# endernewton/tf-faster-rcnn

Hardware: NVIDIA H100
Metric: images/sec (higher is better)
Workload: dtype f16x3 (fp32-grade: fp16 hi/lo split of both operands, 3 wgmma f16 MMAs per product, fp32 accumulate)

## Files before the change

### include/frcnn_b200.h

```cpp
#ifndef FRCNN_B200_H_
#define FRCNN_B200_H_

#include <stddef.h>
#include <stdint.h>

#ifdef __cplusplus
extern "C" {
#endif

typedef enum {
  FRCNN_OK = 0,
  FRCNN_ERR_CUDA = -1,
  FRCNN_ERR_ARG = -2,
  FRCNN_ERR_NO_DEVICE = -3,
  FRCNN_ERR_DRIVER_ENTRY = -4,
  FRCNN_ERR_CAPACITY = -5
} frcnn_status;

#define FRCNN_NMS_PLUS_ONE 1u
#define FRCNN_NMS_INCLUSIVE 2u
#define FRCNN_NMS_SKIP_DEGENERATE 4u
#define FRCNN_NMS_MODE_CPU_NMS (FRCNN_NMS_PLUS_ONE | FRCNN_NMS_INCLUSIVE)
#define FRCNN_NMS_MODE_GPU_NMS (FRCNN_NMS_PLUS_ONE)
#define FRCNN_NMS_MODE_TF (FRCNN_NMS_SKIP_DEGENERATE)
// ... 1 lines not shown
#define FRCNN_ACT_NONE 0
#define FRCNN_ACT_RELU 1
#define FRCNN_ACT_RELU6 2

int frcnn_version(void);
int frcnn_last_error(char* buf, size_t buflen);
int frcnn_check_device(int device_id);
int frcnn_zero_async(void* dev_ptr, size_t bytes, void* stream);

typedef struct frcnn_graph frcnn_graph;
int frcnn_graph_begin(void* stream);
int frcnn_graph_end(void* stream, frcnn_graph** out);
int frcnn_graph_launch(const frcnn_graph* g, void* stream);
void frcnn_graph_destroy(frcnn_graph* g);

int frcnn_nms_host(int* keep_out, int* num_out, const float* boxes_host, int boxes_num, int boxes_dim,
                   float nms_overlap_thresh, int device_id, unsigned flags);

int frcnn_nms_sorted_dev(const float* boxes_dev, int n, float thresh, unsigned flags, int max_out,
                         int* keep_dev, int* num_dev, void* stream);

typedef struct frcnn_conv_plan frcnn_conv_plan;
#define FRCNN_CONV_F16X3 0
#define FRCNN_CONV_TF32X3 1
#define FRCNN_CONV_F16X1 2

typedef struct {
  const float* in_dev;
  const void* w_hi_dev;
  const void* w_lo_dev;
  const float* scale_dev;
  const float* shift_dev;
  const float* residual_dev;
  float* out_dev;
  int n, h, w, cin;
  int cout, kh, kw, stride;
  int pad_t, pad_l;
  int ho, wo;
  int act;
  int block_n;
  int kb_per_chunk;
  int split_k;
  int impl;
  float out_mult;
  const float* in2_dev;
  int cin2;
  float* mean_dev;
  int mean_hw;
} frcnn_conv_desc;

int frcnn_conv_plan_create(frcnn_conv_plan** out, const frcnn_conv_desc* d);
int frcnn_conv_plan_run(const frcnn_conv_plan* p, void* stream);
int frcnn_conv_plan_geometry(const frcnn_conv_desc* d, int sm_count, int* out16);
int frcnn_conv_plan_info(const frcnn_conv_plan* p, int* block_n, int* tile_n, int* tile_h, int* tile_w,
                         int* grid_m, int* grid_n, int* splits, int* smem_bytes);
int frcnn_conv_plan_set_trace(frcnn_conv_plan* p, long long* trace_dev);
void frcnn_conv_plan_destroy(frcnn_conv_plan* p);
int frcnn_debug_watchdog(unsigned int* out16, int reset);

int frcnn_pack_conv_weights(const float* w_hwio_dev, void* w_hi_dev, void* w_lo_dev, int kh, int kw,
                            int cin, int cout, int wexp, void* stream);
int frcnn_pack_conv_weights_tf32(const float* w_hwio_dev, float* w_hi_dev, float* w_lo_dev, int kh, int kw,
                                 int cin, int cout, void* stream);

int frcnn_conv_first(const float* in_dev, const float* w_hwio_dev, const float* scale_dev,
                     const float* shift_dev, float* out_dev, int n, int h, int w, int cout, int k,
                     int stride, int pad_t, int pad_l, int ho, int wo, int act, void* stream);
int frcnn_depthwise3x3(const float* in_dev, const float* w_dev, const float* scale_dev,
                       const float* shift_dev, float* out_dev, int n, int h, int w, int c, int stride,
                       int pad_t, int pad_l, int ho, int wo, int act, void* stream);
int frcnn_max_pool(const float* in_dev, float* out_dev, int n, int h, int w, int c, int k, int stride,
                   int pad_t, int pad_l, int ho, int wo, int pad_is_neg_inf, void* stream);
int frcnn_spatial_mean(const float* in_dev, float* out_dev, int r, int hw, int c, void* stream);

int frcnn_preprocess(const unsigned char* img_dev, int h0, int w0, const double* means3, double fx, double fy,
                     float* blob_dev, int H, int W, void* stream);
int frcnn_preprocess_hflip(const unsigned char* img_dev, int h0, int w0, const double* means3, double fx, double fy,
                           float* blob_dev, int H, int W, void* stream);


int frcnn_rpn_decode(const float* rpn_out_dev, int ld, int delta_col, const float* base_anchors_dev, int num_anchors,
                     int batch, int fh, int fw, int feat_stride, float im_h, float im_w, float* scores_dev,
                     float* props_dev, void* stream);
size_t frcnn_sort_workspace_bytes(int n);
int frcnn_sort_desc(const float* keys_dev, int n, int batch, int* order_dev, float* sorted_keys_dev, void* workspace_dev,
                    size_t workspace_bytes, void* stream);
int frcnn_proposals(const float* props_dev, const float* scores_dev, const int* order_dev, int n, int batch,
                    int pre_nms_top_n, int post_nms_top_n, float thresh, unsigned flags, float* rois_dev,
                    float* roi_scores_dev, int* keep_dev, int* num_dev, void* stream);
int frcnn_crop_pool(const float* feat_dev, int batch, int fh, int fw, int c, const float* rois_dev, int r, int pooled,
                    int pre_pool, float* out_dev, void* stream);
#define FRCNN_ROI_ALIGN_MAX_SAMPLING 16
int frcnn_roi_align(const float* feat_dev, int batch, int fh, int fw, int c, const float* rois_dev, int r, int pooled,
                    float spatial_scale, int sampling_ratio, int aligned, float* out_dev, void* stream);
int frcnn_roi_pool(const float* feat_dev, int batch, int fh, int fw, int c, const float* rois_dev, int r, int pooled,
                   float spatial_scale, float* out_dev, void* stream);
int frcnn_cls_finish(const float* head_out_dev, int ld, int r, int num_classes, const float* stds4,
                     const float* means4, float* cls_score_dev, float* cls_prob_dev, float* bbox_pred_dev,
                     void* stream);
int frcnn_bbox_decode(const float* rois_dev, const float* bbox_pred_dev, int r, int num_classes, int batch,
                      const float* im_meta_dev, float* pred_boxes_dev, void* stream);
size_t frcnn_detect_post_workspace_bytes(int r, int num_classes, int batch);
int frcnn_detect_post(const float* cls_prob_dev, const float* pred_boxes_dev, const int* num_rois_dev, int r, int batch,
                      int num_classes, float score_thresh, float nms_thresh, unsigned flags,
                      int max_per_image, int max_det, float* det_dev, int* ndet_dev, int record_stride, int* keep_dev,
                      int* keep_cnt_dev, float* keep_score_dev, void* workspace_dev, size_t workspace_bytes, void* stream);
// ... 53 lines not shown
```

### tf_faster_rcnn_b200/_native.py

```python
import ctypes as C
import os

_HERE = os.path.dirname(os.path.abspath(__file__))
LIB_PATH = os.path.join(_HERE, "libfrcnn_b200_wd.so" if os.environ.get("FRCNN_LIB_VARIANT") == "wd" else "libfrcnn_b200.so")

NMS_PLUS_ONE, NMS_INCLUSIVE, NMS_SKIP_DEGENERATE = 1, 2, 4
NMS_MODE_CPU_NMS = NMS_PLUS_ONE | NMS_INCLUSIVE
NMS_MODE_GPU_NMS = NMS_PLUS_ONE
NMS_MODE_TF = NMS_SKIP_DEGENERATE
ACT_NONE, ACT_RELU, ACT_RELU6 = 0, 1, 2
CONV_F16X3, CONV_TF32X3, CONV_F16X1 = 0, 1, 2
SOFT_NMS_METHODS = {"linear": 0, "gaussian": 1, "hard": 2}
AUG_MAX_VIEWS = 16
BOX_VOTE_METHODS = {"ID": 0, "AVG": 1, "IOU_AVG": 2, "GENERALIZED_AVG": 3, "QUASI_SUM": 4, "TEMP_AVG": 5}
ROI_ALIGN_MAX_SAMPLING = 16
ROI_MAX_POOLED = 16

vp, ci, cf, cu, sz = C.c_void_p, C.c_int, C.c_float, C.c_uint, C.c_size_t
ip, fp = C.POINTER(C.c_int), C.POINTER(C.c_float)


class ConvDesc(C.Structure):
    _fields_ = [("in_dev", vp), ("w_hi_dev", vp), ("w_lo_dev", vp), ("scale_dev", vp), ("shift_dev", vp),
                ("residual_dev", vp), ("out_dev", vp),
                ("n", ci), ("h", ci), ("w", ci), ("cin", ci), ("cout", ci), ("kh", ci), ("kw", ci), ("stride", ci),
                ("pad_t", ci), ("pad_l", ci), ("ho", ci), ("wo", ci), ("act", ci), ("block_n", ci), ("kb_per_chunk", ci), ("split_k", ci),
                ("impl", ci), ("out_mult", cf), ("in2_dev", vp), ("cin2", ci), ("mean_dev", vp), ("mean_hw", ci)]


SIGNATURES = {
    "frcnn_version": (ci, []),
    "frcnn_last_error": (ci, [C.c_char_p, sz]),
    "frcnn_check_device": (ci, [ci]),
    "frcnn_zero_async": (ci, [vp, sz, vp]),
    "frcnn_graph_begin": (ci, [vp]),
    "frcnn_graph_end": (ci, [vp, C.POINTER(vp)]),
    "frcnn_graph_launch": (ci, [vp, vp]),
    "frcnn_graph_destroy": (None, [vp]),
    "frcnn_nms_host": (ci, [ip, ip, fp, ci, ci, cf, ci, cu]),
    "frcnn_nms_sorted_dev": (ci, [vp, ci, cf, cu, ci, vp, vp, vp]),
    "frcnn_conv_plan_create": (ci, [C.POINTER(vp), C.POINTER(ConvDesc)]),
    "frcnn_conv_plan_run": (ci, [vp, vp]),
    "frcnn_conv_plan_geometry": (ci, [C.POINTER(ConvDesc), ci, ip]),
    "frcnn_conv_plan_info": (ci, [vp, ip, ip, ip, ip, ip, ip, ip, ip]),
    "frcnn_conv_plan_set_trace": (ci, [vp, vp]),
    "frcnn_conv_plan_destroy": (None, [vp]),
    "frcnn_debug_watchdog": (ci, [C.POINTER(C.c_uint), ci]),
    "frcnn_pack_conv_weights": (ci, [vp, vp, vp, ci, ci, ci, ci, ci, vp]),
    "frcnn_pack_conv_weights_tf32": (ci, [vp, vp, vp, ci, ci, ci, ci, vp]),
    "frcnn_conv_first": (ci, [vp, vp, vp, vp, vp, ci, ci, ci, ci, ci, ci, ci, ci, ci, ci, ci, vp]),
    "frcnn_depthwise3x3": (ci, [vp, vp, vp, vp, vp, ci, ci, ci, ci, ci, ci, ci, ci, ci, ci, vp]),
    "frcnn_max_pool": (ci, [vp, vp, ci, ci, ci, ci, ci, ci, ci, ci, ci, ci, ci, vp]),
    "frcnn_spatial_mean": (ci, [vp, vp, ci, ci, ci, vp]),
    "frcnn_preprocess": (ci, [vp, ci, ci, C.POINTER(C.c_double), C.c_double, C.c_double, vp, ci, ci, vp]),
    "frcnn_rpn_decode": (ci, [vp, ci, ci, vp, ci, ci, ci, ci, ci, cf, cf, vp, vp, vp]),
    "frcnn_sort_workspace_bytes": (sz, [ci]),
    "frcnn_sort_desc": (ci, [vp, ci, ci, vp, vp, vp, sz, vp]),
    "frcnn_proposals": (ci, [vp, vp, vp, ci, ci, ci, ci, cf, cu, vp, vp, vp, vp, vp]),
    "frcnn_crop_pool": (ci, [vp, ci, ci, ci, ci, vp, ci, ci, ci, vp, vp]),
    "frcnn_roi_align": (ci, [vp, ci, ci, ci, ci, vp, ci, ci, cf, ci, ci, vp, vp]),
    "frcnn_roi_pool": (ci, [vp, ci, ci, ci, ci, vp, ci, ci, cf, vp, vp]),
    "frcnn_cls_finish": (ci, [vp, ci, ci, ci, fp, fp, vp, vp, vp, vp]),
    "frcnn_bbox_decode": (ci, [vp, vp, ci, ci, ci, vp, vp, vp]),
    "frcnn_detect_post_workspace_bytes": (sz, [ci, ci, ci]),
    "frcnn_detect_regions_workspace_bytes": (ci, [ci, ci, ci, C.POINTER(sz)]),
    "frcnn_detect_post": (ci, [vp, vp, vp, ci, ci, ci, cf, cf, cu, ci, ci, vp, vp, ci, vp, vp, vp, vp, sz, vp]),
    "frcnn_soft_nms_host": (ci, [fp, ip, ip, fp, ci, ci, ci, cf, cf, cf, ci]),
    "frcnn_detect_post_soft": (ci, [vp, vp, vp, ci, ci, ci, cf, ci, cf, cf, cf, ci, ci, vp, vp, ci, vp, vp, vp, vp, sz, vp]),
    "frcnn_detect_features": (ci, [vp, vp, vp, ci, ci, ci, ci, ci, vp, vp, vp]),
    "frcnn_detect_regions": (ci, [vp, vp, vp, vp, vp, ci, ci, ci, ci, cf, cu, cf, ci, ci, vp, vp, vp, vp, sz, vp, vp, vp, vp, vp, vp, vp,
                                  vp, vp]),
    "frcnn_regions_attr_embed": (ci, [vp, ci, ci, ci, vp, vp, ci, vp, ci, vp, vp]),
    "frcnn_attr_finish": (ci, [vp, ci, ci, ci, ci, vp, vp, vp, vp, vp]),
    "frcnn_boxes_to_rois": (ci, [vp, vp, vp, ci, ci, vp, vp, vp]),
    "frcnn_preprocess_hflip": (ci, [vp, ci, ci, C.POINTER(C.c_double), C.c_double, C.c_double, vp, ci, ci, vp]),
    "frcnn_aug_union": (ci, [C.POINTER(vp), C.POINTER(vp), C.POINTER(vp), ip, ip, ci, ci, ci, vp, vp, vp, vp, vp]),
    "frcnn_box_vote_host": (ci, [fp, fp, ci, ci, fp, ci, ci, cf, ci, cf, ci]),
    "frcnn_detect_post_vote": (ci, [vp, vp, vp, ci, ci, ci, cf, cf, cu, ci, ci, vp, vp, ci, vp, vp, vp, vp, sz, cf, ci, cf, vp, vp]),
    "frcnn_detect_post_soft_vote": (ci, [vp, vp, vp, ci, ci, ci, cf, ci, cf, cf, cf, ci, ci, vp, vp, ci, vp, vp, vp, vp, sz, cf, ci, cf, vp,
                                         vp]),
}

_lib = None


def lib():
    global _lib
    if _lib is None:
        if not os.path.exists(LIB_PATH):
            raise RuntimeError("libfrcnn_b200.so not built (%s): the CUDA extension is mandatory, "
                               "there is no CPU fallback" % LIB_PATH)
        L = C.CDLL(LIB_PATH)
        for name, (res, args) in SIGNATURES.items():
            fn = getattr(L, name)
            fn.restype = res
            fn.argtypes = args
# ... 14 lines not shown
```

### tf_faster_rcnn_b200/csrc/conv_gemm.cu

```cuda
#include <cuda_fp16.h>
#include "common.cuh"
#include "../../include/frcnn_b200.h"
#include <stdlib.h>
#include <string.h>

namespace frcnn {

constexpr int BLOCK_M = 128;
constexpr int BLOCK_K = 32;
constexpr int A_TILE_BYTES = BLOCK_M * BLOCK_K * 4;
constexpr int NUM_CONSUMERS = 256;
constexpr int NUM_THREADS = NUM_CONSUMERS + 128;
constexpr int REGS_PRODUCER = 40, REGS_CONSUMER = 232;
constexpr int STAGES = 3;

struct ConvKernelParams {
  float* out;
  const float* residual;
  const float* scale;
  const float* shift;
  int cout, ho, wo, nimg;
  int tn, th, tw;
  int tiles_h, tiles_w;
  int kh, kw, cin, stride, pad_t, pad_l;
  int act;
  int a_box_bytes;
  int kb_per_split;
  int m_tiles, n_tiles, total_units, n_full, splits;
  int raster_n;
  float* ws;
  long long* trace;
  int num_kb_total;
  int cin2;
  float* mean_out;
  float* mean_ws;
  int mean_hw, mean_segs, mean_ld;
};

#ifdef FRCNN_WATCHDOG
#define FRCNN_TRACE(slot, kbv)                                                              \
  do {                                                                                      \
    if (p.trace && blockIdx.x == 0 && (kbv) < 64) p.trace[(kbv) * 8 + (slot)] = clock64(); \
  } while (0)
#else
#define FRCNN_TRACE(slot, kbv) do { } while (0)
#endif

template <int MODE> struct KTraits {
  static constexpr bool TF32 = MODE == FRCNN_CONV_TF32X3;
  static constexpr bool X1 = MODE == FRCNN_CONV_F16X1;
  static constexpr int BOXES = TF32 ? 1 : 2;
  static constexpr int A_BYTES = BOXES * A_TILE_BYTES;
  static constexpr float LO_SCALE = TF32 ? 1.f : 0.00048828125f;
};
template <int BN> constexpr int b_plane_bytes() { return BN * 128; }
template <int BN, int MODE> constexpr int stage_bytes() { return KTraits<MODE>::A_BYTES + 2 * b_plane_bytes<BN>(); }
template <int BN, int MODE> constexpr int smem_bytes() {
  return STAGES * stage_bytes<BN, MODE>() + 1024  + 64 ;
}
constexpr int MEAN_COLS = 64, MEAN_LD = MEAN_COLS + 2;
constexpr int MEAN_SMEM = BLOCK_M * MEAN_LD * 4;
static_assert(smem_bytes<128, FRCNN_CONV_F16X3>() + MEAN_SMEM <= 227 * 1024, "ring exceeds the sm_90 shared-memory limit per block");

struct Unit {
  int w0, h0, n0, nblk, z, kb0, num_kb, slot;
};
__device__ __forceinline__ Unit decode_unit(const ConvKernelParams& p, int u, int num_kb_total) {
  Unit t;
  int tile;
  if (u < p.n_full) { tile = u; t.z = 0; t.slot = -1; }
  else { const int v = u - p.n_full; t.slot = v / p.splits; t.z = v - t.slot * p.splits; tile = p.n_full + t.slot; }
  int mt;
  if (p.raster_n) { t.nblk = tile % p.n_tiles; mt = tile / p.n_tiles; }
  else { mt = tile % p.m_tiles; t.nblk = tile / p.m_tiles; }
  const int tile_w = mt % p.tiles_w;
  const int tile_h = (mt / p.tiles_w) % p.tiles_h;
  const int tile_n = mt / (p.tiles_w * p.tiles_h);
  t.w0 = tile_w * p.tw; t.h0 = tile_h * p.th; t.n0 = tile_n * p.tn;
  if (t.slot < 0) { t.kb0 = 0; t.num_kb = num_kb_total; }
  else { t.kb0 = t.z * p.kb_per_split; t.num_kb = min(p.kb_per_split, num_kb_total - t.kb0); }
  return t;
}

template <int ACT>
__device__ __forceinline__ float apply_act(float a) {
  if (ACT == FRCNN_ACT_RELU) return fmaxf(a, 0.f);
  if (ACT == FRCNN_ACT_RELU6) return fminf(fmaxf(a, 0.f), 6.f);
  return a;
}

template <bool RES, int ACT>
__device__ __forceinline__ float2 finish2(const float2 v, const float2 sc, const float2 sh, const float2 r) {
  float2 y;
  y.x = __fadd_rn(__fmul_rn(v.x, sc.x), sh.x); y.y = __fadd_rn(__fmul_rn(v.y, sc.y), sh.y);
  if (RES) { y.x = __fadd_rn(y.x, r.x); y.y = __fadd_rn(y.y, r.y); }
  y.x = apply_act<ACT>(y.x); y.y = apply_act<ACT>(y.y);
  return y;
}

constexpr int EPI_CHUNK = 8;
template <int BN, bool RES, int ACT>
__device__ __forceinline__ void epilogue_vec(const ConvKernelParams& p, const float (&acc)[BN / 2], const int cbase,
                                             const int pix0, const int pix1) {
  const int cout = p.cout;
  constexpr int NJ = BN / 8;
  constexpr int CH = NJ < EPI_CHUNK ? NJ : EPI_CHUNK;
  static_assert(NJ % CH == 0, "chunking");
  const float* const res0 = RES ? p.residual + (size_t)(pix0 >= 0 ? pix0 : 0) * cout : nullptr;
  const float* const res1 = RES ? p.residual + (size_t)(pix1 >= 0 ? pix1 : 0) * cout : nullptr;
#pragma unroll
  for (int j0 = 0; j0 < NJ; j0 += CH) {
    if (cbase + 8 * j0 >= cout) break;
    float2 sc[CH], sh[CH], r0[CH], r1[CH];
#pragma unroll
    for (int jj = 0; jj < CH; ++jj) {
      const int c = cbase + 8 * (j0 + jj);
      sc[jj] = ld_nc_f2_pinned(p.scale + c);
      sh[jj] = ld_nc_f2_pinned(p.shift + c);
      if (RES) {
        r0[jj] = ld_nc_f2_pinned_if(res0 + c, pix0 >= 0 && c < cout);
        r1[jj] = ld_nc_f2_pinned_if(res1 + c, pix1 >= 0 && c < cout);
      } else {
        r0[jj] = r1[jj] = sc[jj];
      }
    }
#pragma unroll
    for (int jj = 0; jj < CH; ++jj) {
      const int j = j0 + jj;
      const int c = cbase + 8 * j;
      if (c >= cout) break;
      if (pix0 >= 0)
        *reinterpret_cast<float2*>(p.out + (size_t)pix0 * cout + c) =
            finish2<RES, ACT>(make_float2(acc[4 * j], acc[4 * j + 1]), sc[jj], sh[jj], r0[jj]);
      if (pix1 >= 0)
// ... 80 lines not shown
      }
      *reinterpret_cast<float2*>(buf + r0 * MEAN_LD + 8 * jj + 2 * q4) = y0;
      *reinterpret_cast<float2*>(buf + (r0 + 8) * MEAN_LD + 8 * jj + 2 * q4) = y1;
    }
    consumer_bar();
    for (int s = tid / MEAN_COLS; s < nseg; s += NUM_CONSUMERS / MEAN_COLS) {
      const int g = g0 + s;
      const int rs = max(g * hw - t.w0, 0), re = min((g + 1) * hw - t.w0, nrows);
      const float* b = buf + col;
      float a0 = b[rs * MEAN_LD], a1 = 0.f, a2 = 0.f, a3 = 0.f;
      int r = rs + 1;
      for (; r + 3 < re; r += 4) {
        a1 = __fadd_rn(a1, b[r * MEAN_LD]); a2 = __fadd_rn(a2, b[(r + 1) * MEAN_LD]);
        a3 = __fadd_rn(a3, b[(r + 2) * MEAN_LD]); a0 = __fadd_rn(a0, b[(r + 3) * MEAN_LD]);
      }
      for (; r < re; ++r) a1 = __fadd_rn(a1, b[r * MEAN_LD]);
      p.mean_ws[((size_t)mt * p.mean_segs + s) * ld + (size_t)t.nblk * BN + cc + col] = __fadd_rn(__fadd_rn(a0, a1), __fadd_rn(a2, a3));
    }
  }
}

template <int BN>
__device__ __forceinline__ void epilogue_tile(const ConvKernelParams& p, const Unit& t, const float (&acc)[BN / 2], int r0, int q4,
                                              float* mean_buf) {
  if (p.mean_out) {
    epilogue_mean<BN>(p, t, acc, r0, q4, mean_buf);
    return;
  }
  if (t.slot >= 0) {
    float* const w = p.ws + ((size_t)t.slot * p.splits + t.z) * (size_t)(BLOCK_M * BN) + 2 * q4;
#pragma unroll
    for (int j = 0; j < BN / 8; ++j) {
      __stcg(reinterpret_cast<float2*>(w + (size_t)r0 * BN + 8 * j), make_float2(acc[4 * j], acc[4 * j + 1]));
      __stcg(reinterpret_cast<float2*>(w + (size_t)(r0 + 8) * BN + 8 * j), make_float2(acc[4 * j + 2], acc[4 * j + 3]));
    }
    return;
  }
  const int pix0 = tile_pixel(p, t, r0), pix1 = tile_pixel(p, t, r0 + 8);
  const int cbase = t.nblk * BN + 2 * q4;
  if ((p.cout & 3) != 0) {
    epilogue_generic<BN>(p, acc, cbase, pix0, pix1);
    return;
  }
  if (p.residual) epilogue_dispatch<BN, true>(p, acc, cbase, pix0, pix1);
  else epilogue_dispatch<BN, false>(p, acc, cbase, pix0, pix1);
}

template <int BN, int MODE>
__device__ __forceinline__ void wgmma_rs(float (&d)[BN / 2], const uint32_t (&a)[4], uint64_t b_desc, uint32_t scale_d) {
  if (KTraits<MODE>::TF32) wgmma_tf32_rs<BN>(d, a, b_desc, scale_d);
  else wgmma_f16_rs<BN>(d, a, b_desc, scale_d);
}

template <int BN, int MODE>
__global__ void __launch_bounds__(NUM_THREADS, 1)
conv_gemm_kernel(const __grid_constant__ CUtensorMap tmA, const __grid_constant__ CUtensorMap tmA2,
                 const __grid_constant__ CUtensorMap tmBhi, const __grid_constant__ CUtensorMap tmBlo, const ConvKernelParams p) {
  using T = KTraits<MODE>;
  constexpr int kStage = stage_bytes<BN, MODE>();
  constexpr int kPlane = b_plane_bytes<BN>();
  constexpr int NACC = BN / 2;
  static_assert(BN == 64 || BN == 128, "block_n");

  extern __shared__ uint8_t smem_raw[];
  uint8_t* smem = reinterpret_cast<uint8_t*>((reinterpret_cast<uintptr_t>(smem_raw) + 1023) & ~uintptr_t(1023));
  uint64_t* full = reinterpret_cast<uint64_t*>(smem + STAGES * kStage);
  uint64_t* empty = full + STAGES;

  const int warp = threadIdx.x >> 5;
  const int lane = threadIdx.x & 31;
  const int num_kb_total = p.num_kb_total;

  if (threadIdx.x == NUM_CONSUMERS) {
    tma_prefetch_desc(&tmA); tma_prefetch_desc(&tmBhi); tma_prefetch_desc(&tmBlo);
    if (p.cin2) tma_prefetch_desc(&tmA2);
    for (int s = 0; s < STAGES; ++s) { mbar_init(&full[s], 1); mbar_init(&empty[s], NUM_CONSUMERS); }
    mbar_fence_init();
  }
  __syncthreads();
  pdl_launch_dependents();
  pdl_wait();

  if (warp >= NUM_CONSUMERS / 32) {
    reg_dec<REGS_PRODUCER>();
    if (warp == NUM_CONSUMERS / 32 && lane == 0) {
      const int cchunks = p.cin / BLOCK_K;
      const int total1 = p.kh * p.kw * cchunks;
      const int cchunks2 = p.cin2 / BLOCK_K;
      const uint32_t tx = (uint32_t)(T::BOXES * p.a_box_bytes + (T::X1 ? 1 : 2) * kPlane);
      int s = 0; uint32_t ph = 0, kbt = 0;
      for (int u = blockIdx.x; u < p.total_units; u += gridDim.x) {
        const Unit t = decode_unit(p, u, num_kb_total);
#pragma unroll 1
        for (int kb = 0; kb < t.num_kb; ++kb, ++kbt) {
          MBAR_WAIT(&empty[s], ph ^ 1u, 4, kbt);
          uint8_t* st = smem + s * kStage;
          mbar_expect_tx(&full[s], tx);
#pragma unroll
          for (int i = 0; i < T::BOXES; ++i) {
            const int g32 = (t.kb0 + kb) * T::BOXES + i;
            int tap = g32 / cchunks, kc = g32 - tap * cchunks;
            const CUtensorMap* ma = &tmA;
            if (g32 >= total1) {
              tap = 0;
              if (cchunks2) { ma = &tmA2; kc = min(g32 - total1, cchunks2); }
              else kc = cchunks;
            }
            const int r = tap / p.kw, sx = tap - r * p.kw;
            tma_load_4d(st + i * A_TILE_BYTES, ma, &full[s], kc * BLOCK_K, t.w0 * p.stride + sx - p.pad_l,
                        t.h0 * p.stride + r - p.pad_t, t.n0);
          }
          const int kcoord = (t.kb0 + kb) * T::BOXES * BLOCK_K;
          tma_load_2d(st + T::A_BYTES, &tmBhi, &full[s], kcoord, t.nblk * BN);
          if (!T::X1) tma_load_2d(st + T::A_BYTES + kPlane, &tmBlo, &full[s], kcoord, t.nblk * BN);
          FRCNN_TRACE(0, kbt);
          if (++s == STAGES) { s = 0; ph ^= 1u; }
        }
      }
    }
    return;
  }

  reg_inc<REGS_CONSUMER>();
  const int wg = warp >> 2;
  const int q4 = lane & 3;
  const int r0 = wg * 64 + (warp & 3) * 16 + (lane >> 2);
  const uint32_t swz = (uint32_t)(lane >> 2);
  uint32_t aoff[4][2];
#pragma unroll
  for (int j = 0; j < 4; ++j)
#pragma unroll
    for (int h = 0; h < 2; ++h) {
      const int ch = T::TF32 ? j * 8 + h * 4 + q4 : (j & 1) * 16 + h * 8 + 2 * q4;
      const int box = T::TF32 ? 0 : j >> 1;
      aoff[j][h] = (uint32_t)(box * A_TILE_BYTES + r0 * 128) + ((((uint32_t)ch >> 2) ^ swz) << 4) + (((uint32_t)ch & 3u) << 2);
    }
  const uint32_t smem0 = smem_u32(smem);
  int s = 0; uint32_t ph = 0, kbt = 0;
  for (int u = blockIdx.x; u < p.total_units; u += gridDim.x) {
    const Unit t = decode_unit(p, u, num_kb_total);
    float acc[NACC], part[NACC];
#pragma unroll
    for (int i = 0; i < NACC; ++i) { acc[i] = 0.f; part[i] = 0.f; }
#pragma unroll 1
    for (int kb = 0; kb < t.num_kb; ++kb, ++kbt) {
      MBAR_WAIT(&full[s], ph, 1, kbt);
      if (threadIdx.x == 0) FRCNN_TRACE(1, kbt);
      const uint32_t sa = smem0 + (uint32_t)(s * kStage);
      uint32_t ahi[4][4], alo[4][4];
#pragma unroll
      for (int j = 0; j < 4; ++j) {
#pragma unroll
        for (int f = 0; f < 4; ++f) {
          const uint32_t addr = sa + aoff[j][f >> 1] + ((f & 1) ? 1024u : 0u);
          if (T::TF32) {
            float x;
            asm volatile("ld.shared.f32 %0, [%1];" : "=f"(x) : "r"(addr));
            const float hi = to_tf32(x);
            ahi[j][f] = __float_as_uint(hi);
            alo[j][f] = __float_as_uint(to_tf32_fast(__fsub_rn(x, hi)));
          } else {
            float2 x;
            asm volatile("ld.shared.v2.f32 {%0, %1}, [%2];" : "=f"(x.x), "=f"(x.y) : "r"(addr));
            const uint32_t h = pack_f16x2_rn(x.x, x.y);
            const float2 fh = __half22float2(*reinterpret_cast<const __half2*>(&h));
            ahi[j][f] = h;
            alo[j][f] = T::X1 ? 0u : pack_f16x2_rn(__fmul_rn(__fsub_rn(x.x, fh.x), 2048.f), __fmul_rn(__fsub_rn(x.y, fh.y), 2048.f));
          }
        }
      }
      const uint64_t bhi = wgmma_sw128_desc(sa + (uint32_t)T::A_BYTES);
      const uint64_t blo = wgmma_sw128_desc(sa + (uint32_t)(T::A_BYTES + kPlane));
#pragma unroll
      for (int i = 0; i < NACC; ++i) reg_fence(part[i]);
      wgmma_fence();
#pragma unroll
      for (int j = 0; j < 4; ++j) wgmma_rs<BN, MODE>(part, ahi[j], bhi + 2u * j, j > 0 ? 1u : 0u);
      wgmma_commit();
      wgmma_wait_all();
#pragma unroll
      for (int i = 0; i < NACC; ++i) { reg_fence(part[i]); acc[i] = __fadd_rn(acc[i], part[i]); }
      if (!T::X1) {
        wgmma_fence();
#pragma unroll
        for (int j = 0; j < 4; ++j) {
          wgmma_rs<BN, MODE>(part, alo[j], bhi + 2u * j, j > 0 ? 1u : 0u);
          wgmma_rs<BN, MODE>(part, ahi[j], blo + 2u * j, 1u);
        }
        wgmma_commit();
        wgmma_wait_all();
#pragma unroll
        for (int i = 0; i < NACC; ++i) { reg_fence(part[i]); acc[i] = __fmaf_rn(part[i], T::LO_SCALE, acc[i]); }
      }
      mbar_arrive(&empty[s]);
      if (threadIdx.x == 0) FRCNN_TRACE(2, kbt);
      if (++s == STAGES) { s = 0; ph ^= 1u; }
    }
    epilogue_tile<BN>(p, t, acc, r0, q4, reinterpret_cast<float*>(full + 8));
  }
}

template <int BN>
__global__ void __launch_bounds__(256)
tail_reduce_kernel(const ConvKernelParams p) {
  pdl_launch_dependents();
  pdl_wait();
  constexpr int RPB = 256 / (BN / 4);
  constexpr int GROUPS = BLOCK_M / RPB;
  const int slot = blockIdx.x / GROUPS, rgroup = blockIdx.x % GROUPS;
  const int tile = p.n_full + slot;
  const int mt = p.raster_n ? tile / p.n_tiles : tile % p.m_tiles, nblk = p.raster_n ? tile % p.n_tiles : tile / p.m_tiles;
  const int tile_w = mt % p.tiles_w, tile_h = (mt / p.tiles_w) % p.tiles_h, tile_n = mt / (p.tiles_w * p.tiles_h);
  const int rows_img = p.th * p.tw;
  constexpr int C4 = BN / 4;
  static_assert(256 % C4 == 0, "each thread keeps one fixed channel group");
  const float* base = p.ws + (size_t)slot * p.splits * (size_t)(BLOCK_M * BN);
  const bool vec_ok = (p.cout & 3) == 0;
  const int cg = threadIdx.x % C4;
  const int c = nblk * BN + cg * 4;
  if (c >= p.cout) return;
  const float4 sc4 = __ldg(reinterpret_cast<const float4*>(p.scale + c)), sh4 = __ldg(reinterpret_cast<const float4*>(p.shift + c));
  const float sc[4] = {sc4.x, sc4.y, sc4.z, sc4.w}, sh[4] = {sh4.x, sh4.y, sh4.z, sh4.w};
  {
    const int row = rgroup * RPB + threadIdx.x / C4;
    const int dn = row / rows_img, rem = row % rows_img;
    const int n = tile_n * p.tn + dn, h = tile_h * p.th + rem / p.tw, w = tile_w * p.tw + rem % p.tw;
    if (row >= p.tn * rows_img || n >= p.nimg || h >= p.ho || w >= p.wo) return;
    const size_t o = ((((size_t)n * p.ho + h) * p.wo + w)) * p.cout + c;
    float4 rv = make_float4(0.f, 0.f, 0.f, 0.f);
    if (p.residual) {
      if (vec_ok) rv = __ldg(reinterpret_cast<const float4*>(p.residual + o));
      else { float t[4] = {0.f, 0.f, 0.f, 0.f}; for (int e = 0; e < 4; ++e) if (c + e < p.cout) t[e] = __ldg(p.residual + o + e); rv = make_float4(t[0], t[1], t[2], t[3]); }
    }
    float4 a = __ldg(reinterpret_cast<const float4*>(base + (size_t)row * BN) + cg);
    for (int z = 1; z < p.splits; ++z) {
      const float4 b = __ldg(reinterpret_cast<const float4*>(base + ((size_t)z * BLOCK_M + row) * BN) + cg);
      a.x = __fadd_rn(a.x, b.x); a.y = __fadd_rn(a.y, b.y); a.z = __fadd_rn(a.z, b.z); a.w = __fadd_rn(a.w, b.w);
    }
    float y[4] = {a.x, a.y, a.z, a.w};
    const float res[4] = {rv.x, rv.y, rv.z, rv.w};
#pragma unroll
    for (int e = 0; e < 4; ++e) {
      float v = y[e];
      v = __fadd_rn(__fmul_rn(v, sc[e]), sh[e]);
      if (p.residual) v = __fadd_rn(v, res[e]);
      if (p.act == FRCNN_ACT_RELU) v = fmaxf(v, 0.f);
      else if (p.act == FRCNN_ACT_RELU6) v = fminf(fmaxf(v, 0.f), 6.f);
      y[e] = v;
    }
    if (vec_ok) *reinterpret_cast<float4*>(p.out + o) = make_float4(y[0], y[1], y[2], y[3]);
    else for (int e = 0; e < 4; ++e) if (c + e < p.cout) p.out[o + e] = y[e];
  }
// ... 63 lines not shown
    return ERR_CUDA;
  }
  return OK;
}

}

using namespace frcnn;

struct frcnn_conv_plan {
  CUtensorMap tmA, tmA2, tmBhi, tmBlo;
  ConvKernelParams kp;
  int block_n, stages, smem;
  int impl;
  dim3 grid;
  int n_tail;
  float* ws;
  float* eff;
  float* mean_ws;
};

static void choose_tile(int n, int ho, int wo, int stride, int* tn, int* th, int* tw) {
  long best_tiles = -1; int bn = 1, bh = 1, bw = 1; int best_rows = 0;
  const int lim = 256 / stride;
  for (int a = 1; a <= n && a <= BLOCK_M; ++a)
    for (int b = 1; b <= ho && a * b <= BLOCK_M && b <= lim; ++b) {
      int c = BLOCK_M / (a * b);
      if (c > wo) c = wo;
      if (c > lim) c = lim;
      if (c < 1) continue;
      int tiles_w = cdiv(wo, c);
      c = cdiv(wo, tiles_w);
      long tiles = (long)cdiv(n, a) * cdiv(ho, b) * tiles_w;
      int rows = a * b * c;
      if (best_tiles < 0 || tiles < best_tiles || (tiles == best_tiles && rows < best_rows)) {
        best_tiles = tiles; bn = a; bh = b; bw = c; best_rows = rows;
      }
    }
  *tn = bn; *th = bh; *tw = bw;
}

static bool pdl_enabled() {
  static int v = -1;
  if (v < 0) { const char* e = getenv("FRCNN_NO_PDL"); v = (e && e[0] == '1') ? 0 : 1; }
  return v == 1;
}

template <int BN, int MODE>
static int launch(const frcnn_conv_plan* p, cudaStream_t st) {
  static bool attr_done = false;
  if (!attr_done) {
    FRCNN_CUDA(cudaFuncSetAttribute(conv_gemm_kernel<BN, MODE>, cudaFuncAttributeMaxDynamicSharedMemorySize,
                                    smem_bytes<BN, MODE>() + MEAN_SMEM));
    attr_done = true;
  }
  cudaLaunchAttribute attr[1];
  attr[0].id = cudaLaunchAttributeProgrammaticStreamSerialization;
  attr[0].val.programmaticStreamSerializationAllowed = 1;
  const bool pdl = pdl_enabled();
  cudaLaunchConfig_t cfg{};
  cfg.gridDim = p->grid; cfg.blockDim = dim3(NUM_THREADS); cfg.stream = st;
  cfg.dynamicSmemBytes = smem_bytes<BN, MODE>() + (p->kp.mean_out ? MEAN_SMEM : 0);
  cfg.attrs = attr; cfg.numAttrs = pdl ? 1 : 0;
  FRCNN_CUDA(cudaLaunchKernelEx(&cfg, conv_gemm_kernel<BN, MODE>, p->tmA, p->tmA2, p->tmBhi, p->tmBlo, p->kp));
  if (p->kp.mean_out) {
    cudaLaunchConfig_t mc{};
    const long n = (long)(p->kp.wo / p->kp.mean_hw) * p->kp.cout;
    mc.gridDim = dim3((unsigned)((n + 255) / 256)); mc.blockDim = dim3(256); mc.dynamicSmemBytes = 0; mc.stream = st;
    mc.attrs = attr; mc.numAttrs = pdl ? 1 : 0;
    FRCNN_CUDA(cudaLaunchKernelEx(&mc, mean_finish_kernel, p->kp));
  }
  if (p->n_tail > 0) {
    cudaLaunchConfig_t rc{};
    rc.gridDim = dim3((unsigned)(p->n_tail * (BLOCK_M / (256 / (BN / 4))))); rc.blockDim = dim3(256); rc.dynamicSmemBytes = 0; rc.stream = st;
    rc.attrs = attr; rc.numAttrs = pdl ? 1 : 0;
    FRCNN_CUDA(cudaLaunchKernelEx(&rc, tail_reduce_kernel<BN>, p->kp));
  }
  return OK;
}

struct Geometry {
  int n, h, w, ho, wo;
  int tn, th, tw, tiles_w, tiles_h, tiles_n;
  long m_tiles;
  int num_kb, bn, n_tiles, kpc;
  long tiles, n_tail;
  int splits, kbs;
  long total_units;
  int grid;
  int raster_n;
};

static int decide_geometry(const frcnn_conv_desc* d, int sms, Geometry* g) {
  FRCNN_REQUIRE(d->cin > 0 && d->cin % BLOCK_K == 0, "cin=%d must be a positive multiple of 32", d->cin);
  FRCNN_REQUIRE(d->kh >= 1 && d->kw >= 1 && d->stride >= 1 && d->stride <= 8, "bad filter geometry");
  FRCNN_REQUIRE(d->n > 0 && d->h > 0 && d->w > 0 && d->ho > 0 && d->wo > 0 && d->cout > 0, "bad shape");
  FRCNN_REQUIRE(sms > 0, "bad SM count");
  g->n = d->n; g->h = d->h; g->w = d->w; g->ho = d->ho; g->wo = d->wo;
  const bool pointwise = d->kh == 1 && d->kw == 1 && d->stride == 1 && d->pad_t == 0 && d->pad_l == 0 && g->ho == g->h && g->wo == g->w;
  const bool mean = d->mean_hw != 0;
  FRCNN_REQUIRE(d->cin2 >= 0 && d->cin2 % BLOCK_K == 0, "cin2=%d must be 0 or a positive multiple of 32", d->cin2);
  FRCNN_REQUIRE(d->cin2 == 0 || pointwise, "a second A source needs a pointwise layer (1x1, stride 1, no padding)");
  FRCNN_REQUIRE(!mean || pointwise, "the mean epilogue needs a pointwise layer (1x1, stride 1, no padding)");
  FRCNN_REQUIRE(!mean || d->cout % 4 == 0, "the mean epilogue needs cout %% 4 == 0 (cout=%d)", d->cout);
  FRCNN_REQUIRE(d->mean_hw >= 0 && (!mean || ((long)d->n * d->h * d->w) % d->mean_hw == 0),
                "mean_hw=%d must be positive and divide the pixel count", d->mean_hw);
  FRCNN_REQUIRE(!mean || d->split_k <= 1, "the mean epilogue is never split along K");
  if (pointwise) {
    g->w = g->wo = g->n * g->h * g->w; g->n = 1; g->h = g->ho = 1;
  }
  const int ktot = d->kh * d->kw * d->cin + d->cin2;
  choose_tile(g->n, g->ho, g->wo, d->stride, &g->tn, &g->th, &g->tw);
  g->tiles_w = cdiv(g->wo, g->tw); g->tiles_h = cdiv(g->ho, g->th); g->tiles_n = cdiv(g->n, g->tn);
  g->m_tiles = (long)g->tiles_w * g->tiles_h * g->tiles_n;
  const bool f16 = d->impl != FRCNN_CONV_TF32X3;
  const int ks = f16 ? 2 : 1;
  g->num_kb = cdiv(ktot / BLOCK_K, ks);
// ... 2 lines not shown
  if (bn == 0) {
    long best = -1;
    const int cands[2] = {128, 64};
    for (int i = 0; i < 2; ++i) {
      const int c = cands[i];
      if (c > 64 && c / 2 >= d->cout) continue;
      const long ctas = g->m_tiles * cdiv(d->cout, c);
      const long waves = (ctas + sms - 1) / sms;
      const long cost = f16 ? waves * (g->num_kb * 900L + 4000L) : waves * (g->num_kb * 1400L + 6000L);
      if (best < 0 || cost < best) { best = cost; bn = c; }
    }
  }
  FRCNN_REQUIRE(bn == 64 || bn == 128, "block_n must be 64 or 128");
  g->bn = bn;
  g->n_tiles = cdiv(d->cout, bn);
  g->tiles = g->m_tiles * g->n_tiles;
  FRCNN_REQUIRE(g->tiles <= 0x3fffffffL, "too many tiles");
  long n_tail = 0; int splits = 1;
  const int num_kb = g->num_kb;
  const int max_split = num_kb * ks / 8 < 8 ? num_kb * ks / 8 : 8;
  if (d->split_k > 1) {
    n_tail = g->tiles; splits = d->split_k;
  } else if (d->split_k == 0 && max_split >= 2) {
    const long rem = g->tiles % sms;
    if (g->tiles <= sms / 2) { if (num_kb * ks >= 16) { n_tail = g->tiles; splits = (int)(sms / g->tiles); } }
    else if (g->tiles > sms && rem > 0 && rem <= sms / 2 && num_kb * ks >= 48) { n_tail = rem; splits = (int)(sms / rem); }
    if (splits > max_split) splits = max_split;
    if (splits < 2) { n_tail = 0; splits = 1; }
  }
  int kbs = cdiv(num_kb, splits);
  splits = cdiv(num_kb, kbs);
  if (splits < 2 || (d->cout & 3) != 0 || mean) { n_tail = 0; splits = 1; kbs = num_kb; }
  FRCNN_REQUIRE(splits <= 64, "bad split_k");
  g->n_tail = n_tail; g->splits = splits; g->kbs = kbs;
  g->total_units = (g->tiles - n_tail) + n_tail * splits;
  FRCNN_REQUIRE(g->total_units <= 0x7fffffffL, "too many work units");
  g->grid = (int)(g->total_units < sms ? g->total_units : sms);
  {
    const char* e = getenv("FRCNN_CONV_RASTER");
    const double a_bytes = (double)d->n * d->h * d->w * (d->cin + d->cin2) * 4.0, b_bytes = (double)d->cout * ktot * 4.0;
    g->raster_n = (e && (e[0] == 'm' || e[0] == 'n')) ? (e[0] == 'n') : (a_bytes > b_bytes && g->n_tiles > 1);
  }
  return OK;
}

extern "C" int frcnn_conv_plan_geometry(const frcnn_conv_desc* d, int sm_count, int* out16) {
  FRCNN_REQUIRE(d && out16, "null argument");
  Geometry g;
  int rc = decide_geometry(d, sm_count, &g);
  if (rc) return rc;
  const int v[16] = {g.bn, g.tn, g.th, g.tw, (int)g.m_tiles, g.n_tiles, (int)g.tiles, (int)g.n_tail, g.splits, g.kbs,
                     (int)g.total_units, g.grid, g.num_kb, g.kpc, g.tiles_h, g.tiles_w};
  for (int i = 0; i < 16; ++i) out16[i] = v[i];
  return OK;
}

extern "C" int frcnn_conv_plan_create(frcnn_conv_plan** out, const frcnn_conv_desc* d) {
  FRCNN_REQUIRE(out && d, "null argument");
  FRCNN_REQUIRE(d->in_dev && d->w_hi_dev && d->w_lo_dev && (d->mean_hw ? d->mean_dev != nullptr : d->out_dev != nullptr),
                "null device pointer");
  FRCNN_REQUIRE(d->cin2 == 0 || d->in2_dev, "cin2=%d without in2_dev", d->cin2);
  int sms = 132;
  { int dev = 0; cudaDeviceProp pr; if (cudaGetDevice(&dev) == cudaSuccess && cudaGetDeviceProperties(&pr, dev) == cudaSuccess && pr.multiProcessorCount > 0) sms = pr.multiProcessorCount; }
  Geometry g;
  int grc = decide_geometry(d, sms, &g);
  if (grc) return grc;
  frcnn_conv_plan* p = (frcnn_conv_plan*)aligned_alloc(64, (sizeof(frcnn_conv_plan) + 63) / 64 * 64);
  if (!p) { set_error("out of host memory"); return ERR_ARG; }
  memset(p, 0, sizeof(*p));
  const int bn = g.bn;
  {
    uint64_t dims[4] = {(uint64_t)d->cin, (uint64_t)g.w, (uint64_t)g.h, (uint64_t)g.n};
    uint64_t strides[3] = {(uint64_t)d->cin * 4, (uint64_t)g.w * d->cin * 4, (uint64_t)g.h * g.w * d->cin * 4};
    uint32_t box[4] = {(uint32_t)BLOCK_K, (uint32_t)(g.tw * d->stride), (uint32_t)(g.th * d->stride), (uint32_t)g.tn};
    uint32_t es[4] = {1, (uint32_t)d->stride, (uint32_t)d->stride, 1};
    int rc = encode_map(&p->tmA, d->in_dev, 4, dims, strides, box, es);
    if (rc) { free(p); return rc; }
    p->tmA2 = p->tmA;
    if (d->cin2 > 0) {
      uint64_t dims2[4] = {(uint64_t)d->cin2, (uint64_t)g.w, (uint64_t)g.h, (uint64_t)g.n};
      uint64_t strides2[3] = {(uint64_t)d->cin2 * 4, (uint64_t)g.w * d->cin2 * 4, (uint64_t)g.h * g.w * d->cin2 * 4};
      rc = encode_map(&p->tmA2, d->in2_dev, 4, dims2, strides2, box, es);
      if (rc) { free(p); return rc; }
    }
  }
  const bool f16 = d->impl != FRCNN_CONV_TF32X3;
  {
    const uint64_t ktot = (uint64_t)d->kh * d->kw * d->cin + d->cin2;
    uint64_t dims[2] = {ktot, (uint64_t)d->cout};
    uint64_t strides[1] = {ktot * (f16 ? 2 : 4)};
    uint32_t box[2] = {(uint32_t)(f16 ? 2 * BLOCK_K : BLOCK_K), (uint32_t)bn};
    uint32_t es[2] = {1, 1};
    const CUtensorMapDataType dt = f16 ? CU_TENSOR_MAP_DATA_TYPE_FLOAT16 : CU_TENSOR_MAP_DATA_TYPE_FLOAT32;
    const CUtensorMapSwizzle sw = CU_TENSOR_MAP_SWIZZLE_128B;
    int rc = encode_map(&p->tmBhi, d->w_hi_dev, 2, dims, strides, box, es, dt, sw);
    if (!rc) rc = encode_map(&p->tmBlo, d->w_lo_dev, 2, dims, strides, box, es, dt, sw);
    if (rc) { free(p); return rc; }
  }
  ConvKernelParams& k = p->kp;
  k.out = d->out_dev; k.residual = d->residual_dev;
  k.cout = d->cout; k.ho = g.ho; k.wo = g.wo; k.nimg = g.n;
  k.tn = g.tn; k.th = g.th; k.tw = g.tw; k.tiles_h = g.tiles_h; k.tiles_w = g.tiles_w;
  k.kh = d->kh; k.kw = d->kw; k.cin = d->cin; k.stride = d->stride; k.pad_t = d->pad_t; k.pad_l = d->pad_l;
  k.act = d->act;
  k.a_box_bytes = g.tn * g.th * g.tw * BLOCK_K * 4;
  k.trace = nullptr;
  k.num_kb_total = g.num_kb;
  k.m_tiles = (int)g.m_tiles; k.n_tiles = g.n_tiles;
  k.kb_per_split = g.kbs; k.splits = g.splits; k.n_full = (int)(g.tiles - g.n_tail);
  k.total_units = (int)g.total_units;
  k.raster_n = g.raster_n;
  k.cin2 = d->cin2;
  k.mean_out = d->mean_hw ? d->mean_dev : nullptr; k.mean_ws = nullptr; k.mean_hw = d->mean_hw; k.mean_ld = g.n_tiles * bn;
  k.mean_segs = d->mean_hw ? (g.tw < cdiv(g.tw - 1, d->mean_hw) + 1 ? g.tw : cdiv(g.tw - 1, d->mean_hw) + 1) : 0;
  k.ws = nullptr; p->ws = nullptr; p->eff = nullptr; p->mean_ws = nullptr; p->n_tail = (int)g.n_tail;
  {
    const int padded = g.n_tiles * bn;
    const float om = f16 ? (d->out_mult != 0.f ? d->out_mult : 1.f) : 1.f;
    cudaError_t e = cudaMalloc(&p->eff, (size_t)2 * padded * sizeof(float));
    if (e != cudaSuccess) { free(p); return cuda_fail(e, "epilogue vectors", __FILE__, __LINE__); }
    prep_epilogue_vectors_kernel<<<cdiv(padded, 256), 256>>>(d->scale_dev, d->shift_dev, om, d->cout, padded, p->eff, p->eff + padded);
    e = cudaGetLastError();
    if (e == cudaSuccess) e = cudaDeviceSynchronize();
    if (e != cudaSuccess) { cudaFree(p->eff); free(p); return cuda_fail(e, "prep_epilogue_vectors", __FILE__, __LINE__); }
    k.scale = p->eff; k.shift = p->eff + padded;
  }
  if (g.n_tail > 0) {
    cudaError_t e = cudaMalloc(&p->ws, (size_t)g.n_tail * g.splits * BLOCK_M * bn * sizeof(float));
    if (e != cudaSuccess) { cudaFree(p->eff); free(p); return cuda_fail(e, "split-tile workspace", __FILE__, __LINE__); }
    k.ws = p->ws;
  }
  if (d->mean_hw) {
    cudaError_t e = cudaMalloc(&p->mean_ws, (size_t)g.m_tiles * k.mean_segs * k.mean_ld * sizeof(float));
    if (e != cudaSuccess) { cudaFree(p->eff); free(p); return cuda_fail(e, "mean workspace", __FILE__, __LINE__); }
    k.mean_ws = p->mean_ws;
  }
  p->grid = dim3((unsigned)g.grid, 1, 1);
  p->block_n = bn;
  p->impl = f16 ? (d->impl == FRCNN_CONV_F16X1 ? FRCNN_CONV_F16X1 : FRCNN_CONV_F16X3) : FRCNN_CONV_TF32X3;
  p->stages = STAGES;
  p->smem = f16 ? (bn == 128 ? smem_bytes<128, FRCNN_CONV_F16X3>() : smem_bytes<64, FRCNN_CONV_F16X3>())
              : (bn == 128 ? smem_bytes<128, FRCNN_CONV_TF32X3>() : smem_bytes<64, FRCNN_CONV_TF32X3>());
  if (d->mean_hw) p->smem += MEAN_SMEM;
  *out = p;
  return OK;
}

extern "C" int frcnn_conv_plan_run(const frcnn_conv_plan* p, void* stream) {
  FRCNN_REQUIRE(p, "null plan");
  cudaStream_t st = (cudaStream_t)stream;
  if (p->impl == FRCNN_CONV_F16X3) return p->block_n == 128 ? launch<128, FRCNN_CONV_F16X3>(p, st) : launch<64, FRCNN_CONV_F16X3>(p, st);
  if (p->impl == FRCNN_CONV_F16X1) return p->block_n == 128 ? launch<128, FRCNN_CONV_F16X1>(p, st) : launch<64, FRCNN_CONV_F16X1>(p, st);
  return p->block_n == 128 ? launch<128, FRCNN_CONV_TF32X3>(p, st) : launch<64, FRCNN_CONV_TF32X3>(p, st);
}

extern "C" int frcnn_conv_plan_info(const frcnn_conv_plan* p, int* block_n, int* tile_n, int* tile_h, int* tile_w,
                                    int* grid_m, int* grid_n, int* stages, int* smem) {
  FRCNN_REQUIRE(p, "null plan");
  if (block_n) *block_n = p->block_n;
  if (tile_n) *tile_n = p->kp.tn;
  if (tile_h) *tile_h = p->kp.th;
  if (tile_w) *tile_w = p->kp.tw;
  if (grid_m) *grid_m = p->kp.m_tiles;
  if (grid_n) *grid_n = p->kp.n_tiles;
  if (stages) *stages = p->n_tail > 0 ? p->kp.splits : 1;
// ... 31 lines not shown
```

Before: 261.7.

## Skip K-blocks whose filter taps fall entirely in zero padding per tile

Computes, per output tile, which kernel rows and columns touch only padding, and skips the TMA loads and MMAs for K-blocks made up only of those taps. The producer filters K-blocks and the consumer counts live blocks, so both sides stay in step. A separate kernel instantiation is used only when the plan finds at least one unit with dead blocks. This removes wasted MMA work on border tiles at the cost of per-block predicate checks and more code paths.

```diff
diff --git a/include/frcnn_b200.h b/include/frcnn_b200.h
--- a/include/frcnn_b200.h
+++ b/include/frcnn_b200.h
@@ -77,6 +77,7 @@
 int frcnn_conv_plan_create(frcnn_conv_plan** out, const frcnn_conv_desc* d);
 int frcnn_conv_plan_run(const frcnn_conv_plan* p, void* stream);
 int frcnn_conv_plan_geometry(const frcnn_conv_desc* d, int sm_count, int* out16);
+int frcnn_conv_plan_live_kblocks(const frcnn_conv_desc* d, int sm_count, long long* total, int* per_unit);
 int frcnn_conv_plan_info(const frcnn_conv_plan* p, int* block_n, int* tile_n, int* tile_h, int* tile_w,
                          int* grid_m, int* grid_n, int* splits, int* smem_bytes);
 int frcnn_conv_plan_set_trace(frcnn_conv_plan* p, long long* trace_dev);
diff --git a/tf_faster_rcnn_b200/_native.py b/tf_faster_rcnn_b200/_native.py
--- a/tf_faster_rcnn_b200/_native.py
+++ b/tf_faster_rcnn_b200/_native.py
@@ -42,6 +42,7 @@
     "frcnn_conv_plan_create": (ci, [C.POINTER(vp), C.POINTER(ConvDesc)]),
     "frcnn_conv_plan_run": (ci, [vp, vp]),
     "frcnn_conv_plan_geometry": (ci, [C.POINTER(ConvDesc), ci, ip]),
+    "frcnn_conv_plan_live_kblocks": (ci, [C.POINTER(ConvDesc), ci, C.POINTER(C.c_longlong), ip]),
     "frcnn_conv_plan_info": (ci, [vp, ip, ip, ip, ip, ip, ip, ip, ip]),
     "frcnn_conv_plan_set_trace": (ci, [vp, vp]),
     "frcnn_conv_plan_destroy": (None, [vp]),
diff --git a/tf_faster_rcnn_b200/csrc/conv_gemm.cu b/tf_faster_rcnn_b200/csrc/conv_gemm.cu
--- a/tf_faster_rcnn_b200/csrc/conv_gemm.cu
+++ b/tf_faster_rcnn_b200/csrc/conv_gemm.cu
@@ -35,6 +35,8 @@
   float* mean_out;
   float* mean_ws;
   int mean_hw, mean_segs, mean_ld;
+  int h, w;
+  int skip_padding;
 };
 
 #ifdef FRCNN_WATCHDOG
@@ -62,10 +64,28 @@
 constexpr int MEAN_SMEM = BLOCK_M * MEAN_LD * 4;
 static_assert(smem_bytes<128, FRCNN_CONV_F16X3>() + MEAN_SMEM <= 227 * 1024, "ring exceeds the sm_90 shared-memory limit per block");
 
+__host__ __device__ __forceinline__ uint32_t axis_live_taps(int o0, int t, int o_end, int stride, int pad, int extent, int k) {
+  const int last = (o0 + t < o_end ? o0 + t : o_end) - 1;
+  if (stride == 1) {
+    const int lo = pad - last > 0 ? pad - last : 0;
+    const int hi = extent - 1 + pad - o0 < k - 1 ? extent - 1 + pad - o0 : k - 1;
+    return lo > hi ? 0u : (((1u << k) - 1u) >> (k - 1 - hi)) & ~((1u << lo) - 1u);
+  }
+  uint32_t m = 0u;
+#pragma unroll 1
+  for (int r = 0; r < k; ++r) {
+    const int off = r - pad;
+    const int first_in = off < 0 ? (-off + stride - 1) / stride : 0;
+    const int o = o0 > first_in ? o0 : first_in;
+    if (o <= last && o * stride + off < extent) m |= 1u << r;
+  }
+  return m;
+}
+
 struct Unit {
   int w0, h0, n0, nblk, z, kb0, num_kb, slot;
 };
-__device__ __forceinline__ Unit decode_unit(const ConvKernelParams& p, int u, int num_kb_total) {
+__host__ __device__ __forceinline__ Unit decode_unit(const ConvKernelParams& p, int u, int num_kb_total) {
   Unit t;
   int tile;
   if (u < p.n_full) { tile = u; t.z = 0; t.slot = -1; }
@@ -78,8 +98,58 @@
   const int tile_n = mt / (p.tiles_w * p.tiles_h);
   t.w0 = tile_w * p.tw; t.h0 = tile_h * p.th; t.n0 = tile_n * p.tn;
   if (t.slot < 0) { t.kb0 = 0; t.num_kb = num_kb_total; }
-  else { t.kb0 = t.z * p.kb_per_split; t.num_kb = min(p.kb_per_split, num_kb_total - t.kb0); }
+  else { t.kb0 = t.z * p.kb_per_split; t.num_kb = p.kb_per_split < num_kb_total - t.kb0 ? p.kb_per_split : num_kb_total - t.kb0; }
   return t;
+}
+
+struct LiveTaps {
+  uint32_t rows, cols;
+  bool all;
+};
+__host__ __device__ __forceinline__ LiveTaps live_taps(const ConvKernelParams& p, const Unit& t) {
+  LiveTaps m;
+  m.rows = m.cols = ~0u;
+  m.all = true;
+  if (p.skip_padding && (p.kh > 1 || p.kw > 1) && p.kh < 32 && p.kw < 32) {
+    m.rows = axis_live_taps(t.h0, p.th, p.ho, p.stride, p.pad_t, p.h, p.kh);
+    m.cols = axis_live_taps(t.w0, p.tw, p.wo, p.stride, p.pad_l, p.w, p.kw);
+    m.all = m.rows == (1u << p.kh) - 1u && m.cols == (1u << p.kw) - 1u;
+  }
+  return m;
+}
+
+__host__ __device__ __forceinline__ bool kblock_live(const ConvKernelParams& p, const LiveTaps& m, int kb, int boxes) {
+  if (m.all) return true;
+  const int cchunks = p.cin / BLOCK_K, total1 = p.kh * p.kw * cchunks;
+  for (int i = 0; i < boxes; ++i) {
+    const int g32 = kb * boxes + i;
+    if (g32 >= total1) continue;
+    const int tap = g32 / cchunks, r = tap / p.kw, s = tap - r * p.kw;
+    if ((m.rows >> r) & (m.cols >> s) & 1u) return true;
+  }
+  return false;
+}
+
+__host__ __device__ __forceinline__ int live_kblocks(const ConvKernelParams& p, const Unit& t, int boxes) {
+  const LiveTaps m = live_taps(p, t);
+  if (m.all) return t.num_kb;
+  const int cchunks = p.cin / BLOCK_K, end = t.kb0 + t.num_kb;
+  int n = 0;
+  if (cchunks % boxes != 0) {
+#pragma unroll 1
+    for (int kb = t.kb0; kb < end; ++kb) n += kblock_live(p, m, kb, boxes) ? 1 : 0;
+    return n;
+  }
+  const int per_tap = cchunks / boxes;
+#pragma unroll 1
+  for (int r = 0, tap = 0; r < p.kh; ++r)
+#pragma unroll 1
+    for (int s = 0; s < p.kw; ++s, ++tap) {
+      const int lo = tap * per_tap > t.kb0 ? tap * per_tap : t.kb0;
+      const int hi = (tap + 1) * per_tap < end ? (tap + 1) * per_tap : end;
+      if (lo < hi && ((m.rows >> r) & (m.cols >> s) & 1u)) n += hi - lo;
+    }
+  return n;
 }
 
 template <int ACT>
@@ -266,10 +336,9 @@
   else wgmma_f16_rs<BN>(d, a, b_desc, scale_d);
 }
 
-template <int BN, int MODE>
-__global__ void __launch_bounds__(NUM_THREADS, 1)
-conv_gemm_kernel(const __grid_constant__ CUtensorMap tmA, const __grid_constant__ CUtensorMap tmA2,
-                 const __grid_constant__ CUtensorMap tmBhi, const __grid_constant__ CUtensorMap tmBlo, const ConvKernelParams p) {
+template <int BN, int MODE, bool SKIP>
+__device__ __forceinline__ void conv_gemm_body(const CUtensorMap& tmA, const CUtensorMap& tmA2, const CUtensorMap& tmBhi,
+                                               const CUtensorMap& tmBlo, const ConvKernelParams& p) {
   using T = KTraits<MODE>;
   constexpr int kStage = stage_bytes<BN, MODE>();
   constexpr int kPlane = b_plane_bytes<BN>();
@@ -305,8 +374,10 @@
       int s = 0; uint32_t ph = 0, kbt = 0;
       for (int u = blockIdx.x; u < p.total_units; u += gridDim.x) {
         const Unit t = decode_unit(p, u, num_kb_total);
+        const LiveTaps lt = SKIP ? live_taps(p, t) : LiveTaps{~0u, ~0u, true};
 #pragma unroll 1
-        for (int kb = 0; kb < t.num_kb; ++kb, ++kbt) {
+        for (int kb = 0; kb < t.num_kb; ++kb) {
+          if (SKIP && !kblock_live(p, lt, t.kb0 + kb, T::BOXES)) continue;
           MBAR_WAIT(&empty[s], ph ^ 1u, 4, kbt);
           uint8_t* st = smem + s * kStage;
           mbar_expect_tx(&full[s], tx);
@@ -329,6 +400,7 @@
           if (!T::X1) tma_load_2d(st + T::A_BYTES + kPlane, &tmBlo, &full[s], kcoord, t.nblk * BN);
           FRCNN_TRACE(0, kbt);
           if (++s == STAGES) { s = 0; ph ^= 1u; }
+          ++kbt;
         }
       }
     }
@@ -356,8 +428,9 @@
     float acc[NACC], part[NACC];
 #pragma unroll
     for (int i = 0; i < NACC; ++i) { acc[i] = 0.f; part[i] = 0.f; }
+    const int num_live = SKIP ? live_kblocks(p, t, T::BOXES) : t.num_kb;
 #pragma unroll 1
-    for (int kb = 0; kb < t.num_kb; ++kb, ++kbt) {
+    for (int kb = 0; kb < num_live; ++kb, ++kbt) {
       MBAR_WAIT(&full[s], ph, 1, kbt);
       if (threadIdx.x == 0) FRCNN_TRACE(1, kbt);
       const uint32_t sa = smem0 + (uint32_t)(s * kStage);
@@ -412,6 +485,20 @@
     }
     epilogue_tile<BN>(p, t, acc, r0, q4, reinterpret_cast<float*>(full + 8));
   }
+}
+
+template <int BN, int MODE>
+__global__ void __launch_bounds__(NUM_THREADS, 1)
+conv_gemm_kernel(const __grid_constant__ CUtensorMap tmA, const __grid_constant__ CUtensorMap tmA2,
+                 const __grid_constant__ CUtensorMap tmBhi, const __grid_constant__ CUtensorMap tmBlo, const ConvKernelParams p) {
+  conv_gemm_body<BN, MODE, false>(tmA, tmA2, tmBhi, tmBlo, p);
+}
+
+template <int BN, int MODE>
+__global__ void __launch_bounds__(NUM_THREADS, 1)
+conv_gemm_skip_kernel(const __grid_constant__ CUtensorMap tmA, const __grid_constant__ CUtensorMap tmA2,
+                      const __grid_constant__ CUtensorMap tmBhi, const __grid_constant__ CUtensorMap tmBlo, const ConvKernelParams p) {
+  conv_gemm_body<BN, MODE, true>(tmA, tmA2, tmBhi, tmBlo, p);
 }
 
 template <int BN>
@@ -581,6 +668,8 @@
   if (!attr_done) {
     FRCNN_CUDA(cudaFuncSetAttribute(conv_gemm_kernel<BN, MODE>, cudaFuncAttributeMaxDynamicSharedMemorySize,
                                     smem_bytes<BN, MODE>() + MEAN_SMEM));
+    FRCNN_CUDA(cudaFuncSetAttribute(conv_gemm_skip_kernel<BN, MODE>, cudaFuncAttributeMaxDynamicSharedMemorySize,
+                                    smem_bytes<BN, MODE>() + MEAN_SMEM));
     attr_done = true;
   }
   cudaLaunchAttribute attr[1];
@@ -591,7 +680,8 @@
   cfg.gridDim = p->grid; cfg.blockDim = dim3(NUM_THREADS); cfg.stream = st;
   cfg.dynamicSmemBytes = smem_bytes<BN, MODE>() + (p->kp.mean_out ? MEAN_SMEM : 0);
   cfg.attrs = attr; cfg.numAttrs = pdl ? 1 : 0;
-  FRCNN_CUDA(cudaLaunchKernelEx(&cfg, conv_gemm_kernel<BN, MODE>, p->tmA, p->tmA2, p->tmBhi, p->tmBlo, p->kp));
+  if (p->kp.skip_padding) FRCNN_CUDA(cudaLaunchKernelEx(&cfg, conv_gemm_skip_kernel<BN, MODE>, p->tmA, p->tmA2, p->tmBhi, p->tmBlo, p->kp));
+  else FRCNN_CUDA(cudaLaunchKernelEx(&cfg, conv_gemm_kernel<BN, MODE>, p->tmA, p->tmA2, p->tmBhi, p->tmBlo, p->kp));
   if (p->kp.mean_out) {
     cudaLaunchConfig_t mc{};
     const long n = (long)(p->kp.wo / p->kp.mean_hw) * p->kp.cout;
@@ -700,6 +790,45 @@
   const int v[16] = {g.bn, g.tn, g.th, g.tw, (int)g.m_tiles, g.n_tiles, (int)g.tiles, (int)g.n_tail, g.splits, g.kbs,
                      (int)g.total_units, g.grid, g.num_kb, g.kpc, g.tiles_h, g.tiles_w};
   for (int i = 0; i < 16; ++i) out16[i] = v[i];
+  return OK;
+}
+
+static void unit_params(const frcnn_conv_desc* d, const Geometry& g, ConvKernelParams* k) {
+  k->cout = d->cout; k->ho = g.ho; k->wo = g.wo; k->nimg = g.n; k->h = g.h; k->w = g.w;
+  k->tn = g.tn; k->th = g.th; k->tw = g.tw; k->tiles_h = g.tiles_h; k->tiles_w = g.tiles_w;
+  k->kh = d->kh; k->kw = d->kw; k->cin = d->cin; k->stride = d->stride; k->pad_t = d->pad_t; k->pad_l = d->pad_l;
+  k->num_kb_total = g.num_kb;
+  k->m_tiles = (int)g.m_tiles; k->n_tiles = g.n_tiles;
+  k->kb_per_split = g.kbs; k->splits = g.splits; k->n_full = (int)(g.tiles - g.n_tail);
+  k->total_units = (int)g.total_units;
+  k->raster_n = g.raster_n;
+  k->cin2 = d->cin2;
+  k->skip_padding = 1;
+  const int boxes = d->impl == FRCNN_CONV_TF32X3 ? KTraits<FRCNN_CONV_TF32X3>::BOXES : KTraits<FRCNN_CONV_F16X3>::BOXES;
+  bool any = false;
+  for (int u = 0; u < k->total_units && !any; ++u) {
+    const Unit t = decode_unit(*k, u, k->num_kb_total);
+    any = live_kblocks(*k, t, boxes) < t.num_kb;
+  }
+  k->skip_padding = any ? 1 : 0;
+}
+
+extern "C" int frcnn_conv_plan_live_kblocks(const frcnn_conv_desc* d, int sm_count, long long* total, int* per_unit) {
+  FRCNN_REQUIRE(d && total, "null argument");
+  Geometry g;
+  int rc = decide_geometry(d, sm_count, &g);
+  if (rc) return rc;
+  ConvKernelParams k;
+  memset(&k, 0, sizeof(k));
+  unit_params(d, g, &k);
+  const int boxes = d->impl == FRCNN_CONV_TF32X3 ? KTraits<FRCNN_CONV_TF32X3>::BOXES : KTraits<FRCNN_CONV_F16X3>::BOXES;
+  long long sum = 0;
+  for (int u = 0; u < k.total_units; ++u) {
+    const int n = live_kblocks(k, decode_unit(k, u, k.num_kb_total), boxes);
+    if (per_unit) per_unit[u] = n;
+    sum += n;
+  }
+  *total = sum;
   return OK;
 }
 
@@ -746,19 +875,11 @@
     if (rc) { free(p); return rc; }
   }
   ConvKernelParams& k = p->kp;
+  unit_params(d, g, &k);
   k.out = d->out_dev; k.residual = d->residual_dev;
-  k.cout = d->cout; k.ho = g.ho; k.wo = g.wo; k.nimg = g.n;
-  k.tn = g.tn; k.th = g.th; k.tw = g.tw; k.tiles_h = g.tiles_h; k.tiles_w = g.tiles_w;
-  k.kh = d->kh; k.kw = d->kw; k.cin = d->cin; k.stride = d->stride; k.pad_t = d->pad_t; k.pad_l = d->pad_l;
   k.act = d->act;
   k.a_box_bytes = g.tn * g.th * g.tw * BLOCK_K * 4;
   k.trace = nullptr;
-  k.num_kb_total = g.num_kb;
-  k.m_tiles = (int)g.m_tiles; k.n_tiles = g.n_tiles;
-  k.kb_per_split = g.kbs; k.splits = g.splits; k.n_full = (int)(g.tiles - g.n_tail);
-  k.total_units = (int)g.total_units;
-  k.raster_n = g.raster_n;
-  k.cin2 = d->cin2;
   k.mean_out = d->mean_hw ? d->mean_dev : nullptr; k.mean_ws = nullptr; k.mean_hw = d->mean_hw; k.mean_ld = g.n_tiles * bn;
   k.mean_segs = d->mean_hw ? (g.tw < cdiv(g.tw - 1, d->mean_hw) + 1 ? g.tw : cdiv(g.tw - 1, d->mean_hw) + 1) : 0;
   k.ws = nullptr; p->ws = nullptr; p->eff = nullptr; p->mean_ws = nullptr; p->n_tail = (int)g.n_tail;
```

Result: no change. 263.8 (median of 6 runs) (+0.8%).
